# kianmcevoy/audio_analysis

Measured on AMD Instinct MI355X. Metric: IRs/sec full report (STFT+RT60bands+zplane), 48 kHz 10 s IR, higher is better.
Workload: dtype f64; 1 GPU; metrics-only full report on 256 mono synthetic IRs per GPU per step, 10 s @ 48 kHz (SURVEY.md 8d generator), H2D included: every step uploads its batch from pinned host memory (float32, 492 MB) on a copy stream under the previous step's kernels; 4 distinct batches rotate; batch_per_gpu=256, parallelism=file-sharded dp1, gather=final

## Files before the change

audio_analysis_amd/build.py:

```python
from __future__ import annotations

import os
import shutil
import subprocess
import sys
from concurrent.futures import ThreadPoolExecutor
from pathlib import Path

CSRC = Path(__file__).resolve().parent / "csrc"
LIB = CSRC / "libira.so"
ARCH = "gfx950"

SOURCES = {
    "ira_api.hip": [],
    "ira_edc.hip": ["-ffp-contract=off"],
    "ira_stft.hip": ["-fno-slp-vectorize"],
    "ira_stft2.hip": ["-fno-slp-vectorize"],
    "ira_stft3.hip": ["-fno-slp-vectorize"],
    "ira_stft4.hip": [],
    "ira_fftlong.hip": [],
    "ira_fftsmooth.hip": [],
    "ira_spectrum.hip": ["-ffp-contract=off"],
    "ira_modal.hip": ["-ffp-contract=off"],
    "ira_ar.hip": [],
    "ira_ingest.hip": ["-ffp-contract=off"],
    "ira_deconv.hip": ["-ffp-contract=off"],
    "ira_diffusion.hip": ["-ffp-contract=off"],
    "ira_energy.hip": ["-ffp-contract=off"],
}
COMMON = ["-O3", "-std=c++17", "-fPIC", f"--offload-arch={ARCH}", "-Wall", "-Wno-unused-function"]


def _hipcc() -> str:
    exe = shutil.which("hipcc") or "/opt/rocm/bin/hipcc"
    if not Path(exe).exists():
        raise RuntimeError("hipcc not found; libira cannot be built")
    return exe


def _stale(obj: Path, deps) -> bool:
    if not obj.exists():
        return True
    t = obj.stat().st_mtime
    return any(Path(d).stat().st_mtime > t for d in deps)


def build_tuning(verbose: bool = True) -> Path:
    hipcc = _hipcc()
    objs = []
    out = CSRC / "libira_tuning.so"
    tmp = CSRC / "_tuning"
    tmp.mkdir(exist_ok=True)
    for name, extra in SOURCES.items():
        obj = tmp / (Path(name).stem + ".o")
        cmd = [hipcc, *COMMON, "-DIRA_TUNING_BUILD", *extra, "-c", str(CSRC / name), "-o", str(obj)]
        if verbose:
            print(" ".join(cmd), flush=True)
        subprocess.run(cmd, check=True)
        objs.append(obj)
    subprocess.run([hipcc, "-shared", "-fPIC", f"--offload-arch={ARCH}", *map(str, objs), "-o", str(out)], check=True)
    return out


def build(force: bool = False, verbose: bool = False) -> Path:
    hipcc = _hipcc()
    headers = list(CSRC.glob("*.h")) + [CSRC.parent.parent / "include" / "ira.h"]
    jobs = []
    objs = []
    for name, extra in SOURCES.items():
        src = CSRC / name
        obj = CSRC / (src.stem + ".o")
        objs.append(obj)
        if force or _stale(obj, [src, Path(__file__)] + headers):
            jobs.append([hipcc, *COMMON, *extra, "-c", str(src), "-o", str(obj)])

    def run(cmd):
        if verbose:
            print(" ".join(cmd), flush=True)
        r = subprocess.run(cmd, capture_output=True, text=True)
        if r.returncode != 0:
            raise RuntimeError(f"hipcc failed:\n{' '.join(cmd)}\n{r.stdout}\n{r.stderr}")
        if verbose and r.stderr.strip():
            print(r.stderr, flush=True)

    if jobs:
        with ThreadPoolExecutor(max_workers=min(4, len(jobs))) as ex:
            list(ex.map(run, jobs))
    if jobs or force or _stale(LIB, objs):
        run([hipcc, "-shared", "-fPIC", f"--offload-arch={ARCH}", *map(str, objs), "-o", str(LIB)])
    return LIB


if __name__ == "__main__":
    if "--tuning" in sys.argv:
        print(build_tuning())
        sys.exit(0)
    p = build(force="--force" in sys.argv, verbose=True)
    print(p)
```

audio_analysis_amd/csrc/ira_stft4.hip:

```cpp
#include <cmath>
#include <cstdlib>

#include "ira_fft_reg.h"
#include "ira_log.h"
#include "ira_stft.h"

namespace {

using ira::brev_bits;
using ira::cplx;
using ira::dft_dif;
using ira::powers16;

typedef cplx<double> cdd;

constexpr int M4 = 4096, F4 = M4 + 1, TL4 = 128;
constexpr int ROW4 = 129;
constexpr int E2N4 = 256;
constexpr int EXC4 = 16 * ROW4;
static_assert(EXC4 >= 8 * E2N4 && EXC4 * 2 >= M4, "exchange buffer too small");

__device__ __forceinline__ float db_of4(double re, double im, double floor_pow, float floor_db,
                                        const ira::LogTabEntry* tab) {
  const double p = fma(re, re, im * im);
  if (!(p > floor_pow)) return floor_db;
  return (float)(3.0102999566398120 * ira::log2_table<4>(p, tab));
}

__device__ __forceinline__ double lin_of4(double re, double im, double floor_pow, float floor_db, double floor_lin32,
                                          const ira::LogTabEntry* tab) {
  const double p = fma(re, re, im * im);
  if (!(p > floor_pow)) return floor_lin32;
  const double db = 3.0102999566398120 * ira::log2_table<4>(p, tab);
  const double t = ((double)(float)db - db) * 0.11512925464970228;
  const double y0 = __builtin_amdgcn_rsq(p);
  double g = p * y0;
  const double h = 0.5 * y0;
  const double r = fma(-h, g, 0.5);
  g = fma(g, r, g);
  return g * fma(t, fma(t, 0.5, 1.0), 1.0);
}

constexpr int TL5 = 256;

__global__ __launch_bounds__(TL5) __attribute__((amdgpu_waves_per_eu(4, 4))) void stft5_kernel(
    const float* __restrict__ x, const int64_t* __restrict__ off, const int32_t* __restrict__ nframes, int hop,
    const double* __restrict__ window, const cdd* __restrict__ tw, double floor_lin, float floor_db,
    float* __restrict__ out, const int64_t* __restrict__ out_off, const int32_t* __restrict__ frame_sel,
    const int64_t* __restrict__ sel_off, int lb_nbins, int lb_kbase, const int32_t* __restrict__ lb_first,
    const int32_t* __restrict__ lb_count, int ablate) {
  __shared__ __attribute__((aligned(16))) cdd ex[EXC4];
  __shared__ ira::LogTabEntry ltab[ira::LOGTAB_N];
  __shared__ int lb_range[2];
  __shared__ int frame_bad;
  const unsigned gx = gridDim.x, nwg = gridDim.x * gridDim.y;
  const unsigned orig = blockIdx.y * gx + blockIdx.x;
  const unsigned xq = nwg / 8, xr = nwg % 8, xcd = orig % 8;
  const unsigned wg = (xcd < xr ? xcd * (xq + 1) : xr * (xq + 1) + (xcd - xr) * xq) + orig / 8;
  const int seg = (int)(wg / gx);
  const int col = (int)(wg % gx);
  const int T_out = nframes[seg];
  if (col >= T_out) return;
  const int q = threadIdx.x;
  double* exd = reinterpret_cast<double*>(ex);
  ira::build_log_table(ltab, q);
  if (q < 2) lb_range[q] = q == 0 ? F4 : 0;

  const int64_t frame = frame_sel ? (int64_t)frame_sel[sel_off[seg] + col] : (int64_t)col;
  const float* fx = x + off[seg] + frame * hop;
  const int k1l = q & 15, n3l = q >> 4;
  const bool lower = q < TL4;
  cdd wuni[8];
#pragma unroll
  for (int i = 0; i < 8; ++i) wuni[i] = tw[TL5 * i];

  cdd v[16];
  {
    float xa[16], xb[16];
    double wa[16], wb[16];
#pragma unroll
    for (int n1 = 0; n1 < 16; ++n1) {
      const int n = n1 * 256 + q;
      if (IRA_ABL(ablate & 2)) { xa[n1] = (float)(n & 7) * 0.125f; xb[n1] = (float)(q & 3); }
      else { xa[n1] = fx[2 * n]; xb[n1] = fx[2 * n + 1]; }
      if (IRA_ABL(ablate & 1)) { wa[n1] = 0.5 + 1e-4 * n1; wb[n1] = 0.25; }
      else { wa[n1] = window[2 * n]; wb[n1] = window[2 * n + 1]; }
    }
    __builtin_amdgcn_sched_barrier(0);
#pragma unroll
    for (int n1 = 0; n1 < 16; ++n1) v[n1] = {(double)xa[n1] * wa[n1], (double)xb[n1] * wb[n1]};
  }
  dft_dif<double, 16>(v);
  ira::twiddle16<double, true>(v, tw[2 * q]);

  cdd b[16];
  if (lower) {
#pragma unroll
    for (int k1 = 0; k1 < 16; ++k1) ex[k1 * ROW4 + q] = v[brev_bits(k1, 4)];
  }
  __syncthreads();
#pragma unroll
  for (int n2 = 0; n2 < 8; ++n2) b[n2] = ex[k1l * ROW4 + n2 * 16 + n3l];
  __syncthreads();
  if (!lower) {
#pragma unroll
    for (int k1 = 0; k1 < 16; ++k1) ex[k1 * ROW4 + (q - TL4)] = v[brev_bits(k1, 4)];
  }
  __syncthreads();
#pragma unroll
  for (int n2 = 0; n2 < 8; ++n2) b[8 + n2] = ex[k1l * ROW4 + n2 * 16 + n3l];
  __syncthreads();

  dft_dif<double, 16>(b);
  ira::twiddle16<double, true>(b, tw[32 * n3l]);
  if (lower) {
#pragma unroll
    for (int k2 = 0; k2 < 16; ++k2) ex[k1l + 16 * k2 + E2N4 * n3l] = b[brev_bits(k2, 4)];
  }
  __syncthreads();
#pragma unroll
  for (int n3 = 0; n3 < 8; ++n3) v[n3] = ex[q + E2N4 * n3];
  __syncthreads();
  if (!lower) {
#pragma unroll
    for (int k2 = 0; k2 < 16; ++k2) ex[k1l + 16 * k2 + E2N4 * (n3l - 8)] = b[brev_bits(k2, 4)];
  }
  __syncthreads();
#pragma unroll
  for (int n3 = 0; n3 < 8; ++n3) v[8 + n3] = ex[q + E2N4 * n3];
  __syncthreads();

  dft_dif<double, 16>(v);

  double zkr[8], zpr[8], zki[8], zpi[8], midr, midi;
#pragma unroll
  for (int j = 0; j < 8; ++j) ex[j * TL5 + q] = v[brev_bits(8 + j, 4)];
  __syncthreads();
  {
    const int partner = (TL5 - q) & (TL5 - 1);
#pragma unroll
    for (int i = 0; i < 8; ++i) {
      const int slot = q == 0 ? 8 - i : 7 - i;
      cdd zp = v[0];
      if (!(q == 0 && i == 0)) zp = ex[slot * TL5 + partner];
      zkr[i] = v[brev_bits(i, 4)].re; zki[i] = v[brev_bits(i, 4)].im;
      zpr[i] = zp.re; zpi[i] = zp.im;
    }
  }
  {
    const cdd mid = ex[0];
    midr = mid.re; midi = mid.im;
  }
  if (q == 0) frame_bad = !((zkr[0] - zkr[0]) + (zki[0] - zki[0]) == 0.0) ? 1 : 0;
  __syncthreads();
  const bool bad_frame = frame_bad != 0;
  const float qnan32 = __uint_as_float(0x7fc00000u);

  const double floor_pow = floor_lin * floor_lin;
  const cdd wlane = tw[q];
  if (lb_nbins <= 0) {
    float* fo = out + out_off[seg] + (int64_t)col * F4;
#pragma unroll
    for (int i = 0; i < 8; ++i) {
      const int k = q + TL5 * i;
      const cdd e = {0.5 * (zkr[i] + zpr[i]), 0.5 * (zki[i] - zpi[i])};
      const cdd d = {0.5 * (zkr[i] - zpr[i]), 0.5 * (zki[i] + zpi[i])};
      const cdd o = {d.im, -d.re};
      const cdd wk = ira::cmul(wlane, wuni[i]);
      const cdd pp = ira::cmul(wk, o);
      fo[k] = bad_frame ? qnan32 : db_of4(e.re + pp.re, e.im + pp.im, floor_pow, floor_db, ltab);
      fo[M4 - k] = bad_frame ? qnan32 : db_of4(e.re - pp.re, e.im - pp.im, floor_pow, floor_db, ltab);
    }
    if (q == 0) fo[M4 / 2] = bad_frame ? qnan32 : db_of4(midr, midi, floor_pow, floor_db, ltab);
    return;
  }
  {
    int lo = F4, hi = 0;
    for (int bb = q; bb < lb_nbins; bb += TL5) {
      const int c = lb_count[bb];
      if (c > 0) {
        const int f0 = lb_kbase + lb_first[bb];
        lo = f0 < lo ? f0 : lo;
        hi = f0 + c > hi ? f0 + c : hi;
      }
    }
    atomicMin(&lb_range[0], lo);
    atomicMax(&lb_range[1], hi);
  }
  __syncthreads();
  const int k_lo = lb_range[0], k_hi = lb_range[1];
  const double floor_lin32 = exp10((double)floor_db * 0.05);
#pragma unroll
  for (int i = 0; i < 8; ++i) {
    const int k = q + TL5 * i;
    const bool need_a = k >= k_lo && k < k_hi, need_b = (M4 - k) >= k_lo && (M4 - k) < k_hi;
    if (!need_a && !need_b) continue;
    const cdd e = {0.5 * (zkr[i] + zpr[i]), 0.5 * (zki[i] - zpi[i])};
    const cdd d = {0.5 * (zkr[i] - zpr[i]), 0.5 * (zki[i] + zpi[i])};
    const cdd o = {d.im, -d.re};
    const cdd wk = ira::cmul(wlane, wuni[i]);
    const cdd pp = ira::cmul(wk, o);
    if (IRA_ABL(ablate & 4)) {
      if (need_a) exd[k] = e.re + pp.re;
      if (need_b) exd[M4 - k] = e.im - pp.im;
      continue;
    }
    if (need_a) exd[k] = lin_of4(e.re + pp.re, e.im + pp.im, floor_pow, floor_db, floor_lin32, ltab);
    if (need_b) exd[M4 - k] = lin_of4(e.re - pp.re, e.im - pp.im, floor_pow, floor_db, floor_lin32, ltab);
  }
  if (q == 0 && M4 / 2 >= k_lo && M4 / 2 < k_hi) exd[M4 / 2] = lin_of4(midr, midi, floor_pow, floor_db, floor_lin32, ltab);
  __syncthreads();
  float* co = out + out_off[seg];
  for (int bb = q; bb < lb_nbins; bb += TL5) {
    const int c = lb_count[bb];
    float val = qnan32;
    if (c > 0) {
      const double* r = exd + lb_kbase + lb_first[bb];
      double acc = r[0];
      for (int k0 = 1; k0 < c; k0 += 8) {
        double v8[8];
#pragma unroll
        for (int u = 0; u < 8; ++u) v8[u] = (k0 + u < c) ? r[k0 + u] : 0.0;
#pragma unroll
        for (int u = 0; u < 8; ++u)
          if (k0 + u < c) acc += v8[u];
      }
      val = (float)(6.0205999132796239 * ira::log2_table<6>(fmax(acc / (double)c, 1e-30), ltab));
    }
    co[(int64_t)bb * T_out + col] = (bad_frame && c > 0) ? qnan32 : val;
  }
}

}

int32_t ira_stft5_launch(const float* x, const int64_t* off, const int32_t* nframes, int32_t nseg, int32_t max_frames,
                         int32_t hop, const void* window, const void* tw, double floor_db, float* out,
                         const int64_t* out_off, const int32_t* frame_sel, const int64_t* sel_off, int32_t lb_nbins,
                         int32_t lb_kbase, const int32_t* lb_first, const int32_t* lb_count, hipStream_t st) {
  const double floor_lin = std::pow(10.0, floor_db / 20.0);
  dim3 grid(max_frames, nseg);
  stft5_kernel<<<grid, TL5, (size_t)ira_tune_int("IRA_STFT5_LDS_PAD", 0), st>>>(x, off, nframes, hop, static_cast<const double*>(window),
                                     static_cast<const cdd*>(tw), floor_lin, (float)floor_db, out, out_off, frame_sel,
                                     sel_off, lb_nbins, lb_kbase, lb_first, lb_count, ira_tune_int("IRA_STFT5_ABLATE", 0));
  IRA_RETURN_LAUNCH();
}
```

Measured before the change: 14920 IRs/s.

## Process multiple STFT frames per workgroup to amortize setup cost

```diff
diff --git a/audio_analysis_amd/build.py b/audio_analysis_amd/build.py
--- a/audio_analysis_amd/build.py
+++ b/audio_analysis_amd/build.py
@@ -51,13 +51,19 @@
     out = CSRC / "libira_tuning.so"
     tmp = CSRC / "_tuning"
     tmp.mkdir(exist_ok=True)
+    cmds = []
     for name, extra in SOURCES.items():
         obj = tmp / (Path(name).stem + ".o")
-        cmd = [hipcc, *COMMON, "-DIRA_TUNING_BUILD", *extra, "-c", str(CSRC / name), "-o", str(obj)]
+        cmds.append([hipcc, *COMMON, "-DIRA_TUNING_BUILD", *extra, "-c", str(CSRC / name), "-o", str(obj)])
+        objs.append(obj)
+
+    def run(cmd):
         if verbose:
             print(" ".join(cmd), flush=True)
         subprocess.run(cmd, check=True)
-        objs.append(obj)
+
+    with ThreadPoolExecutor(max_workers=4) as ex:
+        list(ex.map(run, cmds))
     subprocess.run([hipcc, "-shared", "-fPIC", f"--offload-arch={ARCH}", *map(str, objs), "-o", str(out)], check=True)
     return out
 
diff --git a/audio_analysis_amd/csrc/ira_stft4.hip b/audio_analysis_amd/csrc/ira_stft4.hip
--- a/audio_analysis_amd/csrc/ira_stft4.hip
+++ b/audio_analysis_amd/csrc/ira_stft4.hip
@@ -42,13 +42,17 @@
 }
 
 constexpr int TL5 = 256;
+constexpr int KF5 = 8;
+
+struct __attribute__((aligned(4))) fpair5 { float a, b; };
+struct __attribute__((aligned(8))) dpair5 { double a, b; };
 
 __global__ __launch_bounds__(TL5) __attribute__((amdgpu_waves_per_eu(4, 4))) void stft5_kernel(
     const float* __restrict__ x, const int64_t* __restrict__ off, const int32_t* __restrict__ nframes, int hop,
     const double* __restrict__ window, const cdd* __restrict__ tw, double floor_lin, float floor_db,
     float* __restrict__ out, const int64_t* __restrict__ out_off, const int32_t* __restrict__ frame_sel,
     const int64_t* __restrict__ sel_off, int lb_nbins, int lb_kbase, const int32_t* __restrict__ lb_first,
-    const int32_t* __restrict__ lb_count, int ablate) {
+    const int32_t* __restrict__ lb_count, int kfr, int ablate) {
   __shared__ __attribute__((aligned(16))) cdd ex[EXC4];
   __shared__ ira::LogTabEntry ltab[ira::LOGTAB_N];
   __shared__ int lb_range[2];
@@ -58,123 +62,24 @@
   const unsigned xq = nwg / 8, xr = nwg % 8, xcd = orig % 8;
   const unsigned wg = (xcd < xr ? xcd * (xq + 1) : xr * (xq + 1) + (xcd - xr) * xq) + orig / 8;
   const int seg = (int)(wg / gx);
-  const int col = (int)(wg % gx);
-  const int T_out = nframes[seg];
-  if (col >= T_out) return;
-  const int q = threadIdx.x;
+  const int col0 = (int)(wg % gx) * kfr;
+  const int T_out = ira::uniform(nframes[seg]);
+  if (col0 >= T_out) return;
+  const int col1 = T_out - col0 < kfr ? T_out : col0 + kfr;
+  int q = threadIdx.x;
   double* exd = reinterpret_cast<double*>(ex);
   ira::build_log_table(ltab, q);
   if (q < 2) lb_range[q] = q == 0 ? F4 : 0;
 
-  const int64_t frame = frame_sel ? (int64_t)frame_sel[sel_off[seg] + col] : (int64_t)col;
-  const float* fx = x + off[seg] + frame * hop;
-  const int k1l = q & 15, n3l = q >> 4;
-  const bool lower = q < TL4;
-  cdd wuni[8];
-#pragma unroll
-  for (int i = 0; i < 8; ++i) wuni[i] = tw[TL5 * i];
-
-  cdd v[16];
-  {
-    float xa[16], xb[16];
-    double wa[16], wb[16];
-#pragma unroll
-    for (int n1 = 0; n1 < 16; ++n1) {
-      const int n = n1 * 256 + q;
-      if (IRA_ABL(ablate & 2)) { xa[n1] = (float)(n & 7) * 0.125f; xb[n1] = (float)(q & 3); }
-      else { xa[n1] = fx[2 * n]; xb[n1] = fx[2 * n + 1]; }
-      if (IRA_ABL(ablate & 1)) { wa[n1] = 0.5 + 1e-4 * n1; wb[n1] = 0.25; }
-      else { wa[n1] = window[2 * n]; wb[n1] = window[2 * n + 1]; }
-    }
-    __builtin_amdgcn_sched_barrier(0);
-#pragma unroll
-    for (int n1 = 0; n1 < 16; ++n1) v[n1] = {(double)xa[n1] * wa[n1], (double)xb[n1] * wb[n1]};
-  }
-  dft_dif<double, 16>(v);
-  ira::twiddle16<double, true>(v, tw[2 * q]);
-
-  cdd b[16];
-  if (lower) {
-#pragma unroll
-    for (int k1 = 0; k1 < 16; ++k1) ex[k1 * ROW4 + q] = v[brev_bits(k1, 4)];
-  }
+  const float* xs = x + ira::uniform(off[seg]);
+  float* os = out + ira::uniform(out_off[seg]);
+  const int32_t* fsel = frame_sel ? frame_sel + ira::uniform(sel_off[seg]) : nullptr;
+  const double floor_pow = floor_lin * floor_lin;
+  const float qnan32 = __uint_as_float(0x7fc00000u);
+  int k_lo = 0, k_hi = 0;
+  double floor_lin32 = 0.0;
   __syncthreads();
-#pragma unroll
-  for (int n2 = 0; n2 < 8; ++n2) b[n2] = ex[k1l * ROW4 + n2 * 16 + n3l];
-  __syncthreads();
-  if (!lower) {
-#pragma unroll
-    for (int k1 = 0; k1 < 16; ++k1) ex[k1 * ROW4 + (q - TL4)] = v[brev_bits(k1, 4)];
-  }
-  __syncthreads();
-#pragma unroll
-  for (int n2 = 0; n2 < 8; ++n2) b[8 + n2] = ex[k1l * ROW4 + n2 * 16 + n3l];
-  __syncthreads();
-
-  dft_dif<double, 16>(b);
-  ira::twiddle16<double, true>(b, tw[32 * n3l]);
-  if (lower) {
-#pragma unroll
-    for (int k2 = 0; k2 < 16; ++k2) ex[k1l + 16 * k2 + E2N4 * n3l] = b[brev_bits(k2, 4)];
-  }
-  __syncthreads();
-#pragma unroll
-  for (int n3 = 0; n3 < 8; ++n3) v[n3] = ex[q + E2N4 * n3];
-  __syncthreads();
-  if (!lower) {
-#pragma unroll
-    for (int k2 = 0; k2 < 16; ++k2) ex[k1l + 16 * k2 + E2N4 * (n3l - 8)] = b[brev_bits(k2, 4)];
-  }
-  __syncthreads();
-#pragma unroll
-  for (int n3 = 0; n3 < 8; ++n3) v[8 + n3] = ex[q + E2N4 * n3];
-  __syncthreads();
-
-  dft_dif<double, 16>(v);
-
-  double zkr[8], zpr[8], zki[8], zpi[8], midr, midi;
-#pragma unroll
-  for (int j = 0; j < 8; ++j) ex[j * TL5 + q] = v[brev_bits(8 + j, 4)];
-  __syncthreads();
-  {
-    const int partner = (TL5 - q) & (TL5 - 1);
-#pragma unroll
-    for (int i = 0; i < 8; ++i) {
-      const int slot = q == 0 ? 8 - i : 7 - i;
-      cdd zp = v[0];
-      if (!(q == 0 && i == 0)) zp = ex[slot * TL5 + partner];
-      zkr[i] = v[brev_bits(i, 4)].re; zki[i] = v[brev_bits(i, 4)].im;
-      zpr[i] = zp.re; zpi[i] = zp.im;
-    }
-  }
-  {
-    const cdd mid = ex[0];
-    midr = mid.re; midi = mid.im;
-  }
-  if (q == 0) frame_bad = !((zkr[0] - zkr[0]) + (zki[0] - zki[0]) == 0.0) ? 1 : 0;
-  __syncthreads();
-  const bool bad_frame = frame_bad != 0;
-  const float qnan32 = __uint_as_float(0x7fc00000u);
-
-  const double floor_pow = floor_lin * floor_lin;
-  const cdd wlane = tw[q];
-  if (lb_nbins <= 0) {
-    float* fo = out + out_off[seg] + (int64_t)col * F4;
-#pragma unroll
-    for (int i = 0; i < 8; ++i) {
-      const int k = q + TL5 * i;
-      const cdd e = {0.5 * (zkr[i] + zpr[i]), 0.5 * (zki[i] - zpi[i])};
-      const cdd d = {0.5 * (zkr[i] - zpr[i]), 0.5 * (zki[i] + zpi[i])};
-      const cdd o = {d.im, -d.re};
-      const cdd wk = ira::cmul(wlane, wuni[i]);
-      const cdd pp = ira::cmul(wk, o);
-      fo[k] = bad_frame ? qnan32 : db_of4(e.re + pp.re, e.im + pp.im, floor_pow, floor_db, ltab);
-      fo[M4 - k] = bad_frame ? qnan32 : db_of4(e.re - pp.re, e.im - pp.im, floor_pow, floor_db, ltab);
-    }
-    if (q == 0) fo[M4 / 2] = bad_frame ? qnan32 : db_of4(midr, midi, floor_pow, floor_db, ltab);
-    return;
-  }
-  {
+  if (lb_nbins > 0) {
     int lo = F4, hi = 0;
     for (int bb = q; bb < lb_nbins; bb += TL5) {
       const int c = lb_count[bb];
@@ -186,48 +91,161 @@
     }
     atomicMin(&lb_range[0], lo);
     atomicMax(&lb_range[1], hi);
+    __syncthreads();
+    k_lo = ira::uniform(lb_range[0]);
+    k_hi = ira::uniform(lb_range[1]);
+    floor_lin32 = ira::uniform(exp10((double)floor_db * 0.05));
   }
-  __syncthreads();
-  const int k_lo = lb_range[0], k_hi = lb_range[1];
-  const double floor_lin32 = exp10((double)floor_db * 0.05);
-#pragma unroll
-  for (int i = 0; i < 8; ++i) {
-    const int k = q + TL5 * i;
-    const bool need_a = k >= k_lo && k < k_hi, need_b = (M4 - k) >= k_lo && (M4 - k) < k_hi;
-    if (!need_a && !need_b) continue;
-    const cdd e = {0.5 * (zkr[i] + zpr[i]), 0.5 * (zki[i] - zpi[i])};
-    const cdd d = {0.5 * (zkr[i] - zpr[i]), 0.5 * (zki[i] + zpi[i])};
-    const cdd o = {d.im, -d.re};
-    const cdd wk = ira::cmul(wlane, wuni[i]);
-    const cdd pp = ira::cmul(wk, o);
-    if (IRA_ABL(ablate & 4)) {
-      if (need_a) exd[k] = e.re + pp.re;
-      if (need_b) exd[M4 - k] = e.im - pp.im;
+
+  for (int col = col0; col < col1; ++col) {
+    asm volatile("" : "+v"(q));
+    const int k1l = q & 15, n3l = q >> 4;
+    const bool lower = q < TL4;
+    const int64_t frame = fsel ? (int64_t)ira::uniform(fsel[col]) : (int64_t)col;
+    const float* fx = xs + frame * hop;
+    int u0 = 0;
+    asm volatile("" : "+s"(u0));
+    cdd wuni[8];
+#pragma unroll
+    for (int i = 0; i < 8; ++i) wuni[i] = tw[TL5 * i + u0];
+
+    cdd v[16];
+    {
+      float xa[16], xb[16];
+      double wa[16], wb[16];
+#pragma unroll
+      for (int n1 = 0; n1 < 16; ++n1) {
+        const int n = n1 * 256 + q;
+        if (IRA_ABL(ablate & 2)) { xa[n1] = (float)(n & 7) * 0.125f; xb[n1] = (float)(q & 3); }
+        else { const fpair5 p = *reinterpret_cast<const fpair5*>(fx + 2 * n); xa[n1] = p.a; xb[n1] = p.b; }
+        if (IRA_ABL(ablate & 1)) { wa[n1] = 0.5 + 1e-4 * n1; wb[n1] = 0.25; }
+        else { const dpair5 w = *reinterpret_cast<const dpair5*>(window + 2 * n); wa[n1] = w.a; wb[n1] = w.b; }
+      }
+      __builtin_amdgcn_sched_barrier(0);
+#pragma unroll
+      for (int n1 = 0; n1 < 16; ++n1) v[n1] = {(double)xa[n1] * wa[n1], (double)xb[n1] * wb[n1]};
+    }
+    dft_dif<double, 16>(v);
+    ira::twiddle16<double, true>(v, tw[2 * q]);
+
+    cdd b[16];
+    if (lower) {
+#pragma unroll
+      for (int k1 = 0; k1 < 16; ++k1) ex[k1 * ROW4 + q] = v[brev_bits(k1, 4)];
+    }
+    __syncthreads();
+#pragma unroll
+    for (int n2 = 0; n2 < 8; ++n2) b[n2] = ex[k1l * ROW4 + n2 * 16 + n3l];
+    __syncthreads();
+    if (!lower) {
+#pragma unroll
+      for (int k1 = 0; k1 < 16; ++k1) ex[k1 * ROW4 + (q - TL4)] = v[brev_bits(k1, 4)];
+    }
+    __syncthreads();
+#pragma unroll
+    for (int n2 = 0; n2 < 8; ++n2) b[8 + n2] = ex[k1l * ROW4 + n2 * 16 + n3l];
+    __syncthreads();
+
+    dft_dif<double, 16>(b);
+    ira::twiddle16<double, true>(b, tw[32 * n3l]);
+    if (lower) {
+#pragma unroll
+      for (int k2 = 0; k2 < 16; ++k2) ex[k1l + 16 * k2 + E2N4 * n3l] = b[brev_bits(k2, 4)];
+    }
+    __syncthreads();
+#pragma unroll
+    for (int n3 = 0; n3 < 8; ++n3) v[n3] = ex[q + E2N4 * n3];
+    __syncthreads();
+    if (!lower) {
+#pragma unroll
+      for (int k2 = 0; k2 < 16; ++k2) ex[k1l + 16 * k2 + E2N4 * (n3l - 8)] = b[brev_bits(k2, 4)];
+    }
+    __syncthreads();
+#pragma unroll
+    for (int n3 = 0; n3 < 8; ++n3) v[8 + n3] = ex[q + E2N4 * n3];
+    __syncthreads();
+
+    dft_dif<double, 16>(v);
+
+    double zkr[8], zpr[8], zki[8], zpi[8], midr, midi;
+#pragma unroll
+    for (int j = 0; j < 8; ++j) ex[j * TL5 + q] = v[brev_bits(8 + j, 4)];
+    __syncthreads();
+    {
+      const int partner = (TL5 - q) & (TL5 - 1);
+#pragma unroll
+      for (int i = 0; i < 8; ++i) {
+        const int slot = q == 0 ? 8 - i : 7 - i;
+        cdd zp = v[0];
+        if (!(q == 0 && i == 0)) zp = ex[slot * TL5 + partner];
+        zkr[i] = v[brev_bits(i, 4)].re; zki[i] = v[brev_bits(i, 4)].im;
+        zpr[i] = zp.re; zpi[i] = zp.im;
+      }
+    }
+    {
+      const cdd mid = ex[0];
+      midr = mid.re; midi = mid.im;
+    }
+    if (q == 0) frame_bad = !((zkr[0] - zkr[0]) + (zki[0] - zki[0]) == 0.0) ? 1 : 0;
+    __syncthreads();
+    const bool bad_frame = frame_bad != 0;
+
+    const cdd wlane = tw[q];
+    if (lb_nbins <= 0) {
+      float* fo = os + (int64_t)col * F4;
+#pragma unroll
+      for (int i = 0; i < 8; ++i) {
+        const int k = q + TL5 * i;
+        const cdd e = {0.5 * (zkr[i] + zpr[i]), 0.5 * (zki[i] - zpi[i])};
+        const cdd d = {0.5 * (zkr[i] - zpr[i]), 0.5 * (zki[i] + zpi[i])};
+        const cdd o = {d.im, -d.re};
+        const cdd wk = ira::cmul(wlane, wuni[i]);
+        const cdd pp = ira::cmul(wk, o);
+        fo[k] = bad_frame ? qnan32 : db_of4(e.re + pp.re, e.im + pp.im, floor_pow, floor_db, ltab);
+        fo[M4 - k] = bad_frame ? qnan32 : db_of4(e.re - pp.re, e.im - pp.im, floor_pow, floor_db, ltab);
+      }
+      if (q == 0) fo[M4 / 2] = bad_frame ? qnan32 : db_of4(midr, midi, floor_pow, floor_db, ltab);
       continue;
     }
-    if (need_a) exd[k] = lin_of4(e.re + pp.re, e.im + pp.im, floor_pow, floor_db, floor_lin32, ltab);
-    if (need_b) exd[M4 - k] = lin_of4(e.re - pp.re, e.im - pp.im, floor_pow, floor_db, floor_lin32, ltab);
-  }
-  if (q == 0 && M4 / 2 >= k_lo && M4 / 2 < k_hi) exd[M4 / 2] = lin_of4(midr, midi, floor_pow, floor_db, floor_lin32, ltab);
-  __syncthreads();
-  float* co = out + out_off[seg];
-  for (int bb = q; bb < lb_nbins; bb += TL5) {
-    const int c = lb_count[bb];
-    float val = qnan32;
-    if (c > 0) {
-      const double* r = exd + lb_kbase + lb_first[bb];
-      double acc = r[0];
-      for (int k0 = 1; k0 < c; k0 += 8) {
-        double v8[8];
-#pragma unroll
-        for (int u = 0; u < 8; ++u) v8[u] = (k0 + u < c) ? r[k0 + u] : 0.0;
-#pragma unroll
-        for (int u = 0; u < 8; ++u)
-          if (k0 + u < c) acc += v8[u];
-      }
-      val = (float)(6.0205999132796239 * ira::log2_table<6>(fmax(acc / (double)c, 1e-30), ltab));
-    }
-    co[(int64_t)bb * T_out + col] = (bad_frame && c > 0) ? qnan32 : val;
+#pragma unroll
+    for (int i = 0; i < 8; ++i) {
+      const int k = q + TL5 * i;
+      const bool need_a = k >= k_lo && k < k_hi, need_b = (M4 - k) >= k_lo && (M4 - k) < k_hi;
+      if (!need_a && !need_b) continue;
+      const cdd e = {0.5 * (zkr[i] + zpr[i]), 0.5 * (zki[i] - zpi[i])};
+      const cdd d = {0.5 * (zkr[i] - zpr[i]), 0.5 * (zki[i] + zpi[i])};
+      const cdd o = {d.im, -d.re};
+      const cdd wk = ira::cmul(wlane, wuni[i]);
+      const cdd pp = ira::cmul(wk, o);
+      if (IRA_ABL(ablate & 4)) {
+        if (need_a) exd[k] = e.re + pp.re;
+        if (need_b) exd[M4 - k] = e.im - pp.im;
+        continue;
+      }
+      if (need_a) exd[k] = lin_of4(e.re + pp.re, e.im + pp.im, floor_pow, floor_db, floor_lin32, ltab);
+      if (need_b) exd[M4 - k] = lin_of4(e.re - pp.re, e.im - pp.im, floor_pow, floor_db, floor_lin32, ltab);
+    }
+    if (q == 0 && M4 / 2 >= k_lo && M4 / 2 < k_hi) exd[M4 / 2] = lin_of4(midr, midi, floor_pow, floor_db, floor_lin32, ltab);
+    __syncthreads();
+    for (int bb = q; bb < lb_nbins; bb += TL5) {
+      const int c = lb_count[bb];
+      float val = qnan32;
+      if (c > 0) {
+        const double* r = exd + lb_kbase + lb_first[bb];
+        double acc = r[0];
+        for (int k0 = 1; k0 < c; k0 += 8) {
+          double v8[8];
+#pragma unroll
+          for (int u = 0; u < 8; ++u) v8[u] = (k0 + u < c) ? r[k0 + u] : 0.0;
+#pragma unroll
+          for (int u = 0; u < 8; ++u)
+            if (k0 + u < c) acc += v8[u];
+        }
+        val = (float)(6.0205999132796239 * ira::log2_table<6>(fmax(acc / (double)c, 1e-30), ltab));
+      }
+      os[(int64_t)bb * T_out + col] = (bad_frame && c > 0) ? qnan32 : val;
+    }
+    __syncthreads();
   }
 }
 
@@ -238,9 +256,11 @@
                          const int64_t* out_off, const int32_t* frame_sel, const int64_t* sel_off, int32_t lb_nbins,
                          int32_t lb_kbase, const int32_t* lb_first, const int32_t* lb_count, hipStream_t st) {
   const double floor_lin = std::pow(10.0, floor_db / 20.0);
-  dim3 grid(max_frames, nseg);
+  int kfr = ira_tune_int("IRA_STFT5_K", KF5);
+  if (kfr < 1) kfr = 1;
+  dim3 grid((max_frames + kfr - 1) / kfr, nseg);
   stft5_kernel<<<grid, TL5, (size_t)ira_tune_int("IRA_STFT5_LDS_PAD", 0), st>>>(x, off, nframes, hop, static_cast<const double*>(window),
                                      static_cast<const cdd*>(tw), floor_lin, (float)floor_db, out, out_off, frame_sel,
-                                     sel_off, lb_nbins, lb_kbase, lb_first, lb_count, ira_tune_int("IRA_STFT5_ABLATE", 0));
+                                     sel_off, lb_nbins, lb_kbase, lb_first, lb_count, kfr, ira_tune_int("IRA_STFT5_ABLATE", 0));
   IRA_RETURN_LAUNCH();
 }
```

After: 15510 IRs/s, median of 6. 1.04x the previous value.
